# syncdoth/face_mask_inpaint

Measured on AMD Instinct MI355X. Metric: train images/sec at 256x256 bs=8 per GPU (PICNet-ref train step), higher is better.
Workload: dtype f32; 1 GPU; train_reference_fill.py PICNet-ref 256x256 fp32, bs=8 per GPU, synthetic CelebA-HQ-shaped batch + random binary_map (BASELINE configs[1]); global_batch=8, parallelism=dp1

## Files before the change

face_mask_inpaint_amd/csrc/conv.hip:

```cpp
#include "gemm_core.h"
#include "conv3x3.h"
#include "conv_p3.h"
#include "convt3x3.h"

static bool aligned16(const void* p) { return ((uintptr_t)p & 15) == 0; }
static int ep_vec(const ConvEp& ep, int Nout) {
  return Nout % 4 == 0 && ep.cstride % 4 == 0 && aligned16(ep.y) && aligned16(ep.bias) && aligned16(ep.res) && aligned16(ep.mask);
}

static int check_desc(const fmi_conv_desc* d) {
  if (!d) return FMI_ERR_BAD_ARG;
  if (d->N <= 0 || d->H <= 0 || d->W <= 0 || d->C <= 0 || d->K <= 0 || d->kh <= 0 || d->kw <= 0 || d->stride <= 0 ||
      d->pad < 0 || d->x_cstride < d->C || d->y_cstride < d->K)
    return FMI_ERR_BAD_ARG;
  const int pe = d->pad, dl = d->dil > 1 ? d->dil : 1;
  if (d->dil < 0 || (dl > 1 && d->pad_mode)) return FMI_ERR_BAD_ARG;
  if (d->OH != (d->H + 2 * pe - dl * (d->kh - 1) - 1) / d->stride + 1 || d->OW != (d->W + 2 * pe - dl * (d->kw - 1) - 1) / d->stride + 1)
    return FMI_ERR_BAD_ARG;
  if (d->OH <= 0 || d->OW <= 0) return FMI_ERR_BAD_ARG;
  if (d->pad_mode == 1 && (d->pad >= d->H || d->pad >= d->W)) return FMI_ERR_UNSUPPORTED;
  if (d->pad_mode != 0 && d->pad_mode != 1) return FMI_ERR_UNSUPPORTED;
  if ((int64_t)d->N * d->H * d->W > 0x7fffffffLL / 2 || (int64_t)d->kh * d->kw * d->C > 0x3fffffffLL) return FMI_ERR_UNSUPPORTED;
  return FMI_OK;
}

static ConvGeom fwd_geom(const fmi_conv_desc* d, const float* x, int n_eff) {
  ConvGeom g{};
  g.N = n_eff; g.IH = d->H; g.IW = d->W; g.C = d->C; g.cstride = d->x_cstride;
  g.GH = d->OH; g.GW = d->OW; g.S = d->stride;
  const int dl = d->dil > 1 ? d->dil : 1;
  g.nty = d->kh; g.ntx = d->kw; g.dy0 = -d->pad; g.dx0 = -d->pad; g.ystep = dl; g.xstep = dl;
  g.kh0 = 0; g.kw0 = 0; g.khstep = 1; g.kwstep = 1; g.kw = d->kw;
  g.pad_mode = d->pad_mode;
  g.vec = (d->C % 4 == 0) && (d->x_cstride % 4 == 0) && aligned16(x);
  g.dGW = make_fastdiv(g.GW); g.dG = make_fastdiv(g.GH * g.GW); g.dC = make_fastdiv(g.C); g.dntx = make_fastdiv(g.ntx);
  g.img_bs = (int64_t)d->H * d->W * d->x_cstride;
  return g;
}

static ConvGeom adj_geom(const fmi_conv_desc* d, const float* dy, int n_eff, int py, int px) {
  const int s = d->stride, dl = d->dil > 1 ? d->dil : 1;
  ConvGeom g{};
  g.N = n_eff; g.IH = d->OH; g.IW = d->OW; g.C = d->K; g.cstride = d->y_cstride;
  g.GH = (d->H - py + s - 1) / s; g.GW = (d->W - px + s - 1) / s; g.S = 1;
  g.kh0 = (py + d->pad) % s; g.kw0 = (px + d->pad) % s;
  g.nty = g.kh0 < d->kh ? (d->kh - g.kh0 + s - 1) / s : 0;
  g.ntx = g.kw0 < d->kw ? (d->kw - g.kw0 + s - 1) / s : 0;
  g.dy0 = (py + d->pad - g.kh0) / s; g.dx0 = (px + d->pad - g.kw0) / s;
  g.ystep = -dl; g.xstep = -dl; g.khstep = s; g.kwstep = s; g.kw = d->kw;
  g.pad_mode = 0;
  g.vec = (d->K % 4 == 0) && (d->y_cstride % 4 == 0) && aligned16(dy);
  g.dGW = make_fastdiv(g.GW); g.dG = make_fastdiv(g.GH * g.GW); g.dC = make_fastdiv(g.C);
  g.dntx = make_fastdiv(g.ntx > 0 ? g.ntx : 1);
  g.img_bs = (int64_t)d->OH * d->OW * d->y_cstride;
  if (g.nty == 0 || g.ntx == 0) { g.nty = 0; g.ntx = 1; }
  return g;
}

#ifndef FMI_HOST_EMU
__global__ void __launch_bounds__(256) conv_split_init_kernel(float* __restrict__ y, const float* __restrict__ bias,
                                                             const float* __restrict__ res, int K, int cstride, int64_t total) {
  for (int64_t i = (int64_t)blockIdx.x * 256 + threadIdx.x; i < total; i += (int64_t)gridDim.x * 256) {
    const int k = (int)(i % K);
    const int64_t o = (i / K) * cstride + k;
    float v = bias ? bias[k] : 0.f;
    if (res) v += res[o];
    y[o] = v;
  }
}
#endif

static int conv_ksplit(int64_t M, int N, int K) {
#ifdef FMI_HOST_EMU
  return 1;
#else
  const int64_t tiles = ceil_div64(M, 128) * ceil_div64(N, N <= 32 ? 32 : (N <= 64 ? 64 : 128));
  if (K < 512 || fmi_det()) return 1;
  if (tiles >= 320) {
    if (tiles >= 800 || K < 2304) return 1;
    return tiles <= 520 ? 2 : 3;
  }
  if (tiles >= 192 && K < 4608) return 1;
  int64_t ks = ceil_div64(384, tiles);
  const int64_t kmin = (M <= 128 && tiles <= 16) ? 64 : 256;
  if (ks > K / kmin) ks = K / kmin;
  return ks < 2 ? 1 : (int)(ks > (kmin == 64 ? 64 : 16) ? (kmin == 64 ? 64 : 16) : ks);
#endif
}

static int conv_phase(const fmi_conv_desc* d, const ConvGeom& g, const float* x, const void* x3, const float* w, const void* w3p,
                      int64_t w_bstride, int Nout, int flip, ConvEp ep, int batch_w, bool may_split, bool shared_init, hipStream_t st) {
  ConvK la{x, g};
  ConvWX lb{w, g, w_bstride, Nout, (Nout % 4 == 0) && aligned16(w) && (w_bstride % 4 == 0)};
  const int ks = may_split ? conv_ksplit(g.Mdim(), Nout, g.Kdim()) : 1;
#ifndef FMI_HOST_EMU
  if (shared_init || ks > 1) {
    if (!shared_init) {
      const int64_t total = (int64_t)g.N * ep.OHt * ep.OWt * Nout;
      hipLaunchKernelGGL(conv_split_init_kernel, dim3(fmi_bw_grid(total, 256)), dim3(256), 0, st, ep.y, ep.bias, ep.res, Nout, ep.cstride,
                         total);
    }
    ep.bias = nullptr;
    ep.res = nullptr;
    ep.act = 3;
    ep.vec = 0;
  }
  const uint16_t* w3 = (const uint16_t*)w3p;
  const int64_t w3_stride = (int64_t)d->kh * d->kw * d->C * d->K;
  const int64_t pixels = (int64_t)g.N * g.IH * g.IW;
  const bool tap3 = d->kh == 3 && d->kw == 3 && d->stride == 1 && d->pad == 1 && d->dil <= 1 && g.pad_mode == 0;
  const bool p3 = batch_w == 1 && g.cstride == g.C && g.Kdim() > 0 && p3_generic_ok(g, x3, w3, Nout);
  if (p3 && tap3 && conv3x3_p3_eligible(x3, w3, g.C, Nout, pixels)) {
    const C3P3Args ca{(const uint16_t*)x3, w3, g.N, g.IH, g.IW, g.C, Nout, flip, make_fastdiv(g.IW), make_fastdiv(g.IH * g.IW)};
    return launch_conv3x3_p3(ca, ep, g.Mdim(), ks, st);
  }
  if (p3)
    return launch_gemm_p3(ConvK3{(const uint16_t*)x3, g, make_fastdiv(g.ntaps())}, ConvWX3{w3, g, w3_stride, Nout}, ep, g.Mdim(), Nout,
                          g.Kdim(), ks, st);
  if (batch_w == 1 && tap3 && conv3x3_eligible(x, w, g.C, g.cstride, Nout, pixels)) {
    const C3Args ca{x, w, g.N, g.IH, g.IW, g.C, g.cstride, Nout, flip, make_fastdiv(g.IW), make_fastdiv(g.IH * g.IW), w3};
    return launch_conv3x3(ca, ep, g.Mdim(), ks, st);
  }
  if (w3 && la.dma_ok()) return launch_gemm(la, ConvWX3{w3, g, w3_stride, Nout}, ep, g.Mdim(), Nout, g.Kdim(), 1, ks, st);
#endif
  return launch_gemm(la, lb, ep, g.Mdim(), Nout, g.Kdim(), batch_w, ks, st);
}

static const void* weight_pieces(const fmi_conv_desc* d, int batch_w, int red_c) {
#ifndef FMI_HOST_EMU
  if (FMI_X6 && batch_w == 1 && red_c % 16 == 0 && aligned16(d->w3)) return d->w3;
#endif
  return nullptr;
}

static int check_y3(const fmi_conv_desc* d, int out_c, int out_cs) {
  if (!d->y3) return FMI_OK;
  return (out_c % 16 == 0 && out_cs == out_c && aligned16(d->y3)) ? FMI_OK : FMI_ERR_BAD_ARG;
}

extern "C" int fmi_conv2d_fwd_f32(const fmi_conv_desc* d, const float* x, const float* wf, const float* bias,
                                  const float* residual, float* y, int act, int batch_w, int64_t w_bstride,
                                  void* stream) {
  if (!d) return FMI_ERR_BAD_ARG;
  int rc = check_y3(d, d->K, d->y_cstride);
  if (rc) return rc;
  rc = check_desc(d);
  if (rc) return rc;
  if (!x || !wf || !y || batch_w < 1 || act < 0 || act > 2) return FMI_ERR_BAD_ARG;
  if (batch_w > 1 && batch_w != d->N) return FMI_ERR_BAD_ARG;
  auto finish = [&](int rc) {
#ifndef FMI_HOST_EMU
    if (rc == FMI_OK && d->y3) rc = fmi_split3_f32(y, d->y3, nullptr, (int64_t)d->N * d->OH * d->OW, d->K, 0, 0.f, stream);
#endif
    return rc;
  };
#ifndef FMI_HOST_EMU
  if (batch_w == 1 && fmi_conv2d_thin_supported(d) && aligned16(x))
    return finish(fmi_conv2d_thin_fwd_f32(d, x, wf, bias, residual, y, act, stream));
#endif
  const ConvGeom g = fwd_geom(d, x, batch_w > 1 ? 1 : d->N);
  const void* w3 = weight_pieces(d, batch_w, d->C);
  ConvEp ep{y, bias, residual, d->OH, d->OW, 1, 0, 0, d->OH, d->OW, d->y_cstride, act, g.dGW, g.dG, (int64_t)d->OH * d->OW * d->y_cstride};
  ep.vec = ep_vec(ep, d->K);
  return finish(conv_phase(d, g, x, d->x3, wf, w3, w_bstride, d->K, 0, ep, batch_w, act == 0 && batch_w == 1, false, (hipStream_t)stream));
}

static int dgrad_impl(const fmi_conv_desc* d, const float* dy, const float* wt, const float* bias, const float* residual,
                      const float* mask, float mslope, float* dx, int batch_w, int64_t w_bstride, void* stream) {
  if (!d) return FMI_ERR_BAD_ARG;
  int rc = check_y3(d, d->C, d->x_cstride);
  if (rc) return rc;
  rc = check_desc(d);
  if (rc) return rc;
  if (!dy || !wt || !dx || batch_w < 1) return FMI_ERR_BAD_ARG;
  if (d->pad_mode != 0) return FMI_ERR_UNSUPPORTED;
  if (batch_w > 1 && batch_w != d->N) return FMI_ERR_BAD_ARG;
  if (mask && bias) return FMI_ERR_UNSUPPORTED;
  auto finish = [&](int rc) {
#ifndef FMI_HOST_EMU
    if (rc == FMI_OK && d->y3) rc = fmi_split3_f32(dx, d->y3, nullptr, (int64_t)d->N * d->H * d->W, d->C, 0, 0.f, stream);
#endif
    return rc;
  };
#ifndef FMI_HOST_EMU
  if (batch_w == 1 && !bias && !residual && !mask && fmi_conv2d_thin_supported(d) && aligned16(dx))
    return finish(fmi_conv2d_thin_dgrad_f32(d, dy, wt, dx, stream));
  if (batch_w == 1 && !bias && !residual && !mask && d->C <= 4 && d->x_cstride == d->C) {
    const int rc_thin = fmi_conv2d_thin_input_dgrad_f32(d, dy, wt, dx, stream);
    if (rc_thin != FMI_ERR_UNSUPPORTED) return finish(rc_thin);
  }
#endif
  const int n_eff = batch_w > 1 ? 1 : d->N;
  const int s = d->stride;
  const void* w3 = weight_pieces(d, batch_w, d->K);
  if (d->dil > 1 && s != 1) return FMI_ERR_UNSUPPORTED;
  bool strided_split = false;
#ifndef FMI_HOST_EMU
  if (s > 1 && batch_w == 1) {
    for (int py = 0; py < s && !strided_split; ++py)
      for (int px = 0; px < s && !strided_split; ++px) {
        const ConvGeom g = adj_geom(d, dy, n_eff, py, px);
        if (g.GH > 0 && g.GW > 0 && conv_ksplit(g.Mdim(), d->C, g.Kdim()) > 1) strided_split = true;
      }
    if (strided_split) {
      const int64_t total = (int64_t)d->N * d->H * d->W * d->C;
      hipLaunchKernelGGL(conv_split_init_kernel, dim3(fmi_bw_grid(total, 256)), dim3(256), 0, (hipStream_t)stream, dx, bias, residual, d->C,
                         d->x_cstride, total);
    }
  }
  if (batch_w == 1 && !strided_split && !d->x3 && convt3x3_eligible(d, dy, (const uint16_t*)w3)) {
    CT3Args ca{};
    ca.x = dy; ca.w3 = (const uint16_t*)w3; ca.N = d->N; ca.H = d->OH; ca.W = d->OW; ca.Cred = d->K; ca.cs = d->y_cstride; ca.Nout = d->C;
    ca.dW = make_fastdiv(d->OW); ca.dHW = make_fastdiv(d->OH * d->OW);
    ConvEp ep{dx, bias, residual, d->OH, d->OW, 2, 0, 0, d->H, d->W, d->x_cstride, 0, ca.dW, ca.dHW, (int64_t)d->H * d->W * d->x_cstride};
    ep.mask = mask;
    ep.mslope = mslope;
    ep.vec = ep_vec(ep, d->C);
    ca.ep = ep;
    return finish(launch_convt3x3(ca, d->N * d->OH * d->OW, (hipStream_t)stream));
  }
#endif
  for (int py = 0; py < s; ++py) {
    for (int px = 0; px < s; ++px) {
      const ConvGeom g = adj_geom(d, dy, n_eff, py, px);
      if (g.GH <= 0 || g.GW <= 0) continue;
      ConvEp ep{dx, bias, residual, g.GH, g.GW, s, py, px, d->H, d->W, d->x_cstride, 0, g.dGW, g.dG,
                (int64_t)d->H * d->W * d->x_cstride};
      ep.mask = mask;
      ep.mslope = mslope;
      ep.vec = ep_vec(ep, d->C);
      rc = conv_phase(d, g, dy, d->x3, wt, w3, w_bstride, d->C, 1, ep, batch_w, batch_w == 1 && (s == 1 || strided_split), strided_split,
                      (hipStream_t)stream);
      if (rc) return rc;
    }
  }
  return finish(FMI_OK);
}
extern "C" int fmi_conv2d_dgrad_f32(const fmi_conv_desc* d, const float* dy, const float* wt, const float* bias,
                                    const float* residual, float* dx, int batch_w, int64_t w_bstride, void* stream) {
  return dgrad_impl(d, dy, wt, bias, residual, nullptr, 0.f, dx, batch_w, w_bstride, stream);
}
extern "C" int fmi_conv_transpose2d_pair_f32(const fmi_conv_desc* d, const float* x1, const float* x2, int K2, const void* w3b,
                                             const float* bias, float* y, void* stream) {
  int rc = check_desc(d);
  if (rc) return rc;
  if (!x1 || !x2 || !w3b || !d->w3 || !y || K2 <= 0) return FMI_ERR_BAD_ARG;
#ifndef FMI_HOST_EMU
  const uint16_t* w3 = (FMI_X6 && d->K % 16 == 0 && aligned16(d->w3)) ? (const uint16_t*)d->w3 : nullptr;
  if (!convt3x3_eligible(d, x1, w3) || (K2 & 15) || !aligned16(x2) || !aligned16(w3b) || d->pad_mode != 0 || d->x3) return FMI_ERR_UNSUPPORTED;
  CT3Args ca{};
  ca.x = x1; ca.w3 = w3; ca.x2 = x2; ca.w3b = (const uint16_t*)w3b; ca.Cred2 = K2; ca.cs2 = K2;
  ca.N = d->N; ca.H = d->OH; ca.W = d->OW; ca.Cred = d->K; ca.cs = d->y_cstride; ca.Nout = d->C;
  ca.dW = make_fastdiv(d->OW); ca.dHW = make_fastdiv(d->OH * d->OW);
  ConvEp ep{y, bias, nullptr, d->OH, d->OW, 2, 0, 0, d->H, d->W, d->x_cstride, 0, ca.dW, ca.dHW, (int64_t)d->H * d->W * d->x_cstride};
  ep.vec = ep_vec(ep, d->C);
  ca.ep = ep;
  return launch_convt3x3(ca, d->N * d->OH * d->OW, (hipStream_t)stream);
#else
  return FMI_ERR_UNSUPPORTED;
#endif
}
extern "C" int fmi_conv2d_dgrad_masked_f32(const fmi_conv_desc* d, const float* dy, const float* wt, const float* mask, float mask_slope,
                                           float* dx, void* stream) {
  if (!mask) return FMI_ERR_BAD_ARG;
  return dgrad_impl(d, dy, wt, nullptr, nullptr, mask, mask_slope, dx, 1, 0, stream);
}

extern "C" int fmi_conv2d_dgrad_masked_add_f32(const fmi_conv_desc* d, const float* dy, const float* wt, const float* mask, float mask_slope,
                                               const float* gadd, float* dx, void* stream) {
  if (!mask || !gadd) return FMI_ERR_BAD_ARG;
  return dgrad_impl(d, dy, wt, nullptr, gadd, mask, mask_slope, dx, 1, 0, stream);
}

extern "C" int fmi_conv2d_wgrad_f32(const fmi_conv_desc* d, const float* x, const float* dy, float* dwf, float* dbias,
                                    int batch_w, int64_t w_bstride, void* stream) {
  int rc = check_desc(d);
  if (rc) return rc;
  if (!x || !dy || !dwf || batch_w < 1) return FMI_ERR_BAD_ARG;
  if (batch_w > 1 && batch_w != d->N) return FMI_ERR_BAD_ARG;
#ifndef FMI_HOST_EMU
  if (batch_w == 1 && fmi_conv2d_thin_supported(d) && aligned16(x)) return fmi_conv2d_thin_wgrad_f32(d, x, dy, dwf, dbias, stream);
#endif
#ifndef FMI_HOST_EMU
  if (FMI_X6 && batch_w == 1 && !dbias && wgrad_p3_ok(d, d->x3, d->y3))
    return launch_wgrad_p3(d, (const uint16_t*)d->x3, (const uint16_t*)d->y3, dwf, (hipStream_t)stream);
#endif
  const int n_eff = batch_w > 1 ? 1 : d->N;
  ConvGeom g = fwd_geom(d, x, n_eff);
  const bool fuse_bias = dbias && batch_w == 1 && (g.Kdim() % 4 == 0);
  if (dbias && !fuse_bias) return FMI_ERR_UNSUPPORTED;
  const int ones_row = fuse_bias ? g.Kdim() : -1;
  const int Mg = g.Kdim() + (fuse_bias ? 1 : 0), Ng = d->K, Kg = g.Mdim();
  WgradAX la{x, g, ones_row};
  DenseX lb{dy, (int64_t)d->y_cstride, (int64_t)d->OH * d->OW * d->y_cstride, Ng, Kg,
            (d->K % 4 == 0) && (d->y_cstride % 4 == 0) && aligned16(dy)};
  WgradEp ep{dwf, g, d->K, w_bstride, dbias, ones_row};
  const int64_t tiles = ceil_div64(Mg, 128) * ceil_div64(Ng, Ng <= 32 ? 32 : (Ng <= 64 ? 64 : 128));
  int64_t ksplit = 2048 / (tiles * batch_w);
  const int64_t kmax = Kg / 512;
  if (ksplit > kmax) ksplit = kmax;
  if (ksplit < 1) ksplit = 1;
  if (fmi_det()) ksplit = 1;
  if (ksplit * batch_w > 65535) ksplit = 65535 / batch_w;
  return launch_gemm(la, lb, ep, Mg, Ng, Kg, batch_w, (int)ksplit, (hipStream_t)stream);
}

#ifndef FMI_HOST_EMU
__global__ void __launch_bounds__(256) bias_grad_vec_f64_kernel(const float* __restrict__ g, int64_t rows, int K4, float* __restrict__ dbias) {
  __shared__ double part[256][4];
  const int cg = threadIdx.x % K4, rl = threadIdx.x / K4, RL = 256 / K4;
  double s[4] = {0, 0, 0, 0};
  for (int64_t r = rl; r < rows; r += RL) {
    const float4 v = reinterpret_cast<const float4*>(g)[r * K4 + cg];
    s[0] += v.x, s[1] += v.y, s[2] += v.z, s[3] += v.w;
  }
#pragma unroll
  for (int e = 0; e < 4; ++e) part[threadIdx.x][e] = s[e];
  __syncthreads();
  if (threadIdx.x < K4) {
    double t[4] = {0, 0, 0, 0};
    for (int l = 0; l < RL; ++l)
#pragma unroll
      for (int e = 0; e < 4; ++e) t[e] += part[l * K4 + threadIdx.x][e];
#pragma unroll
    for (int e = 0; e < 4; ++e) atomicAdd(dbias + 4 * threadIdx.x + e, (float)t[e]);
  }
}
__global__ void __launch_bounds__(256) bias_grad_vec_kernel(const float* __restrict__ g, int64_t rows, int K4,
                                                            float* __restrict__ dbias, int64_t rows_per_block) {
  __shared__ float4 part[256];
  const int cg = threadIdx.x % K4, rl = threadIdx.x / K4, RL = 256 / K4;
  const int64_t r0 = (int64_t)blockIdx.x * rows_per_block;
  int64_t r1 = r0 + rows_per_block;
  if (r1 > rows) r1 = rows;
  float4 s = make_float4(0.f, 0.f, 0.f, 0.f);
  int64_t r = r0 + rl;
  for (; r + 3 * RL < r1; r += 4 * RL) {
    const float4 v0 = reinterpret_cast<const float4*>(g)[r * K4 + cg];
    const float4 v1 = reinterpret_cast<const float4*>(g)[(r + RL) * K4 + cg];
    const float4 v2 = reinterpret_cast<const float4*>(g)[(r + 2 * RL) * K4 + cg];
    const float4 v3 = reinterpret_cast<const float4*>(g)[(r + 3 * RL) * K4 + cg];
    s.x += (v0.x + v1.x) + (v2.x + v3.x);
    s.y += (v0.y + v1.y) + (v2.y + v3.y);
    s.z += (v0.z + v1.z) + (v2.z + v3.z);
    s.w += (v0.w + v1.w) + (v2.w + v3.w);
  }
  for (; r < r1; r += RL) {
    const float4 v = reinterpret_cast<const float4*>(g)[r * K4 + cg];
    s.x += v.x; s.y += v.y; s.z += v.z; s.w += v.w;
  }
  part[threadIdx.x] = s;
  __syncthreads();
  if (threadIdx.x < K4) {
    float4 t = part[threadIdx.x];
    for (int l = 1; l < RL; ++l) {
      const float4 v = part[l * K4 + threadIdx.x];
      t.x += v.x; t.y += v.y; t.z += v.z; t.w += v.w;
    }
    atomicAdd(dbias + 4 * threadIdx.x + 0, t.x);
    atomicAdd(dbias + 4 * threadIdx.x + 1, t.y);
    atomicAdd(dbias + 4 * threadIdx.x + 2, t.z);
    atomicAdd(dbias + 4 * threadIdx.x + 3, t.w);
  }
}
__global__ void __launch_bounds__(256) bias_grad_kernel(const float* __restrict__ g, int64_t rows, int K, int cstride,
                                                        float* __restrict__ dbias, int64_t rows_per_block) {
  __shared__ float part[4][64];
  const int tx = threadIdx.x & 63, ty = threadIdx.x >> 6;
  const int64_t r0 = (int64_t)blockIdx.x * rows_per_block;
  int64_t r1 = r0 + rows_per_block;
  if (r1 > rows) r1 = rows;
  for (int cg = 0; cg < K; cg += 64) {
    const int c = cg + tx;
    float s = 0.f;
    if (c < K)
      for (int64_t r = r0 + ty; r < r1; r += 4) s += g[r * cstride + c];
    part[ty][tx] = s;
    __syncthreads();
    if (ty == 0 && c < K) atomicAdd(dbias + c, part[0][tx] + part[1][tx] + part[2][tx] + part[3][tx]);
    __syncthreads();
  }
}

extern "C" int fmi_bias_grad_f32(const float* g, int64_t rows, int K, int cstride, float* dbias, void* stream) {
  if (!g || !dbias || rows <= 0 || K <= 0 || cstride < K) return FMI_ERR_BAD_ARG;
  int64_t blocks = ceil_div64(rows, 256);
  if (blocks > 256) blocks = 256;
  if (fmi_det()) blocks = 1;
  const int64_t rpb = ceil_div64(rows, blocks);
  blocks = ceil_div64(rows, rpb);
  const int K4 = K / 4;
  if (fmi_det() && K % 4 == 0 && cstride == K && K4 <= 256 && (K4 & (K4 - 1)) == 0 && (((uintptr_t)g) & 15) == 0)
    hipLaunchKernelGGL(bias_grad_vec_f64_kernel, dim3(1), dim3(256), 0, (hipStream_t)stream, g, rows, K4, dbias);
  else if (K % 4 == 0 && cstride == K && K4 <= 256 && (K4 & (K4 - 1)) == 0 && (((uintptr_t)g) & 15) == 0)
    hipLaunchKernelGGL(bias_grad_vec_kernel, dim3((unsigned)blocks), dim3(256), 0, (hipStream_t)stream, g, rows, K4, dbias, rpb);
  else
    hipLaunchKernelGGL(bias_grad_kernel, dim3((unsigned)blocks), dim3(256), 0, (hipStream_t)stream, g, rows, K, cstride, dbias, rpb);
  return fmi_launch_status();
}

__global__ void __launch_bounds__(256) reflect_fold_kernel(const float* __restrict__ gp, float* __restrict__ gx, int N,
                                                           int H, int W, int C, int pad, int64_t total) {
  const int HP = H + 2 * pad, WP = W + 2 * pad;
  for (int64_t i = (int64_t)blockIdx.x * 256 + threadIdx.x; i < total; i += (int64_t)gridDim.x * 256) {
    const int c = (int)(i % C);
    int64_t r = i / C;
    const int x = (int)(r % W);
    r /= W;
    const int y = (int)(r % H);
    const int n = (int)(r / H);
    int ys[3], xs[3], ny = 0, nx = 0;
    ys[ny++] = y + pad;
    if (y >= 1 && y <= pad) ys[ny++] = pad - y;
    if (y <= H - 2 && y >= H - 1 - pad) ys[ny++] = 2 * H - 2 - y + pad;
    xs[nx++] = x + pad;
    if (x >= 1 && x <= pad) xs[nx++] = pad - x;
    if (x <= W - 2 && x >= W - 1 - pad) xs[nx++] = 2 * W - 2 - x + pad;
    float s = 0.f;
    for (int a = 0; a < ny; ++a)
      for (int b = 0; b < nx; ++b) s += gp[(((int64_t)n * HP + ys[a]) * WP + xs[b]) * C + c];
    gx[i] = s;
  }
}

extern "C" int fmi_reflect_pad_fold_f32(const float* gpad, float* gx, int N, int H, int W, int C, int pad, void* stream) {
  if (!gpad || !gx || N <= 0 || H <= 0 || W <= 0 || C <= 0 || pad < 0 || pad >= H || pad >= W) return FMI_ERR_BAD_ARG;
  const int64_t total = (int64_t)N * H * W * C;
  hipLaunchKernelGGL(reflect_fold_kernel, dim3(fmi_bw_grid(total, 256)), dim3(256), 0, (hipStream_t)stream, gpad, gx, N,
                     H, W, C, pad, total);
  return fmi_launch_status();
}
#endif
```

face_mask_inpaint_amd/functional.py:

```python
from __future__ import annotations

import ctypes as C
import math
from typing import List, Optional, Sequence, Tuple

import torch

from . import _lib
from ._lib import ConvDesc, FmiError

EW_LRELU, EW_LRELU_BWD, EW_TANH_BWD, EW_ADD, EW_SCALE, EW_AXPY, EW_MUL, EW_RELU_BWD_OUT, EW_SOFTPLUS, EW_SOFTPLUS_BWD, EW_SUB, EW_RSQRT, EW_RSQRT_BWD, EW_SIGMOID, EW_SIGMOID_BWD = range(15)
ACT_NONE, ACT_TANH, ACT_RELU = 0, 1, 2

ATTN_CHUNK_BYTES = 96 * 1024 * 1024

PROFILE = None


class _prof:
    def __init__(self, tag, flops):
        self.tag, self.flops = tag, flops

    def __enter__(self):
        if PROFILE is not None:
# ... 52 lines not shown


def _p(t: Optional[torch.Tensor], off: int = 0):
    if t is None:
        return None
    return C.c_void_p(t.data_ptr() + 4 * off)


def _chk(*ts, dtype=torch.float32):
    for t in ts:
        if t is None:
            continue
        if not t.is_cuda:
            raise FmiError("face_mask_inpaint_amd ops need device tensors (there is no CPU fallback)")
        if t.dtype != dtype:
            raise FmiError(f"expected {dtype}, got {t.dtype}")
        if not t.is_contiguous():
            raise FmiError("expected a contiguous tensor")


class deterministic:

    def __init__(self, on: bool = True):
        self.on = bool(on)

    def __enter__(self):
        self.prev = _L().set_deterministic(1 if self.on else 0)
        return self

    def __exit__(self, *exc):
        _L().set_deterministic(self.prev)
        return False


def to_nhwc(x: torch.Tensor) -> torch.Tensor:
    return x.permute(0, 2, 3, 1).contiguous()


def to_nchw(x: torch.Tensor) -> torch.Tensor:
    return x.permute(0, 3, 1, 2)


def gemm_raw(a_ptr, b_ptr, c_ptr, M, N, K, sa, sb, sc, batch=1, bs=(0, 0, 0), alpha=1.0, beta=0.0, bias=None, tag="gemm"):
    with _prof(f"{tag}|{M}x{N}x{K} b{batch}", 2.0 * M * N * K * batch):
        _L().gemm_f32(a_ptr, b_ptr, c_ptr, M, N, K, sa[0], sa[1], sb[0], sb[1], sc[0], sc[1], batch, bs[0], bs[1], bs[2],
                      alpha, beta, _p(bias), _st())


def eltwise(op: int, a: torch.Tensor, b: Optional[torch.Tensor] = None, p0: float = 0.0, out: Optional[torch.Tensor] = None):
    _chk(a, b)
    y = torch.empty_like(a) if out is None else out
    if a.numel():
        _L().eltwise_f32(op, _p(a), _p(b), _p(y), a.numel(), float(p0), _st())
    return y


def conv_desc(n, h, w, c, k, kh, kw, stride, pad, pad_mode=0, x_cs=None, y_cs=None, dil=1, w3=None, x3=None) -> Tuple[ConvDesc, int, int]:
    oh = (h + 2 * pad - dil * (kh - 1) - 1) // stride + 1
    ow = (w + 2 * pad - dil * (kw - 1) - 1) // stride + 1
    d = ConvDesc(n, h, w, c, oh, ow, k, x_cs or c, y_cs or k, kh, kw, stride, pad, pad_mode, dil)
    if w3 is not None:
        d.w3 = w3.data_ptr()
        if x3 is not None:
            d.x3 = x3.data_ptr()
    return d, oh, ow


P3_ENABLED = True
P3_MIN_PIXELS = 16384
P3_MIN_WORK = 1152
P3_MIN_COUT = 64


def p3_wanted(pixels: int, cred: int, cout: int, taps: int) -> bool:
    return P3_ENABLED and cred % 16 == 0 and cred >= 64 and cout >= P3_MIN_COUT and pixels >= P3_MIN_PIXELS and taps * cout >= P3_MIN_WORK


def p3_of(t: torch.Tensor, lrelu_from: Optional[torch.Tensor] = None, slope: float = 0.0, colsum: Optional[list] = None) -> Optional[torch.Tensor]:
    c = t.shape[-1]
    if c % 16 or t.dtype != torch.float32 or not t.is_cuda or not t.is_contiguous() or t.data_ptr() % 16:
        if lrelu_from is not None:
            eltwise(EW_LRELU, lrelu_from, None, slope, out=t)
        return None
    p = getattr(t, "_fmi_p3", None)
    if p is not None and p[1] == t._version and lrelu_from is None:
        return p[0]
    x3 = torch.empty(t.numel() * 3, device=t.device, dtype=torch.bfloat16)
    if lrelu_from is not None:
        _L().split3_f32(_p(lrelu_from), C.c_void_p(x3.data_ptr()), _p(t), t.numel() // c, c, 1, float(slope), _st())
    elif colsum is not None and c <= 512 and 256 % (c // 8) == 0 and not _L().get_deterministic():
        gb = _zeros(c, t.device, torch.float32)
        _L().split3_colsum_f32(_p(t), C.c_void_p(x3.data_ptr()), _p(gb), t.numel() // c, c, _st())
        colsum.append(gb)
    else:
        _L().split3_f32(_p(t), C.c_void_p(x3.data_ptr()), None, t.numel() // c, c, 0, 0.0, _st())
    t._fmi_p3 = (x3, t._version)
    return x3


class PackedWeight:

    __slots__ = ("wf", "wt", "rows", "C", "kh", "kw", "w3")

    def __init__(self, wf, wt, rows, Cc, kh, kw, w3=(None, None)):
        self.wf, self.wt, self.rows, self.C, self.kh, self.kw = wf, wt, rows, Cc, kh, kw
        self.w3 = w3


W3_ENABLED = True
_LAST_W3: List[Tuple[Optional[torch.Tensor], Optional[torch.Tensor]]] = []


class _WeightPrepare(torch.autograd.Function):

    @staticmethod
    def forward(ctx, metas, *ws):
        lib = _L()
        n = len(ws)
        dev = ws[0].device
        sig = torch.ones(n, device=dev, dtype=torch.float32)
        entries = (_lib.WeightEntry * n)()
        wfs, wts, w3s = [], [], []
        for i, (w, meta) in enumerate(zip(ws, metas)):
            u, v = meta[0], meta[1]
            want_w3 = meta[2] if len(meta) > 2 else True
            iters = int(meta[3]) if len(meta) > 3 else 1
            _chk(w, u, v)
            rows, cc, kh, kw = w.shape
            if u is not None and rows > 4096:
                raise FmiError("spectral-norm weight with more than 4096 rows")
            wf = torch.empty((kh * kw, cc, rows), device=dev, dtype=torch.float32)
            wt = torch.empty((kh * kw, rows, cc), device=dev, dtype=torch.float32)
            pieces = W3_ENABLED and want_w3 and kh * kw <= 36 and w.is_cuda
            wf3 = torch.empty(3 * kh * kw * cc * rows, device=dev, dtype=torch.bfloat16) if pieces and cc % 16 == 0 else None
            wt3 = torch.empty(3 * kh * kw * cc * rows, device=dev, dtype=torch.bfloat16) if pieces and rows % 16 == 0 else None
            w3s.append((wf3, wt3))
            e = entries[i]
            e.wf3 = wf3.data_ptr() if wf3 is not None else None
            e.wt3 = wt3.data_ptr() if wt3 is not None else None
            e.w = w.data_ptr()
            e.u = u.data_ptr() if u is not None else None
            e.v = v.data_ptr() if v is not None else None
            e.wf, e.wt = wf.data_ptr(), wt.data_ptr()
            e.sigma = sig.data_ptr() + 4 * i
            e.rows, e.C, e.taps, e.iters = rows, cc, kh * kw, iters
            wfs.append(wf)
            wts.append(wt)
        lib.weight_prepare_f32(entries, n, _st())
        ctx.metas, ctx.ws, ctx.sig = metas, ws, sig
        _LAST_W3[:] = w3s
        ctx.mark_non_differentiable(sig, *wts)
        ctx.set_materialize_grads(False)
        return (sig,) + tuple(wfs) + tuple(wts)

    @staticmethod
    def backward(ctx, _gsig, *gs):
        lib = _L()
        n = len(ctx.ws)
        gwf = gs[:n]
        live = [i for i, g in enumerate(gwf) if g is not None and ctx.needs_input_grad[1 + i]]
        grads: List[Optional[torch.Tensor]] = [None] * n
        if live:
            entries = (_lib.WeightGradEntry * len(live))()
            keep = []
            for j, i in enumerate(live):
                w = ctx.ws[i]
                u, v = ctx.metas[i][0], ctx.metas[i][1]
                g = gwf[i].contiguous()
                dw = torch.empty_like(w)
                keep.append(g)
                e = entries[j]
                e.w = w.data_ptr()
                e.u = u.data_ptr() if u is not None else None
                e.v = v.data_ptr() if v is not None else None
                e.sigma = ctx.sig.data_ptr() + 4 * i
                e.dwf = g.data_ptr()
                e.dw = dw.data_ptr()
                e.rows, e.C, e.taps = w.shape[0], w.shape[1], w.shape[2] * w.shape[3]
                grads[i] = dw
            scratch = _zeros(len(live), ctx.sig.device, torch.float32)
            lib.weight_grad_f32(entries, len(live), _p(scratch), _st())
        return (None,) + tuple(grads)


def prepare_weights(items: Sequence[tuple]) -> List[PackedWeight]:
    metas = tuple(tuple(it[1:]) for it in items)
    ws = tuple(it[0] for it in items)
    n = len(ws)
    res = _WeightPrepare.apply(metas, *ws)
    w3s = list(_LAST_W3)
    _LAST_W3.clear()
    return [PackedWeight(res[1 + i], res[1 + n + i], w.shape[0], w.shape[1], w.shape[2], w.shape[3], w3s[i]) for i, w in enumerate(ws)]


def _act_bwd(g, y, act):
    if act == ACT_TANH:
        return eltwise(EW_TANH_BWD, g, y)
    if act == ACT_RELU:
        return eltwise(EW_RELU_BWD_OUT, g, y)
    return g


class _Conv2d(torch.autograd.Function):

    @staticmethod
    def forward(ctx, x, wf, bias, residual, wt, kh, kw, stride, pad, pad_mode, act, in_act=None, skip_act_bwd=False, dil=1, passthrough=False, w3=(None, None)):
        _chk(x, wf, bias, residual)
        lib = _L()
        x_in = x
        n, h, w, c = x.shape
        k = wf.shape[2]
        use3 = w3[0] is not None and pad_mode == 0 and p3_wanted(n * h * w, c, k, kh * kw)
        x3 = None
        if in_act is not None and in_act[0] == "apply":
            if use3:
                x = torch.empty_like(x_in)
                x3 = p3_of(x, lrelu_from=x_in, slope=in_act[1])
            else:
                x = eltwise(EW_LRELU, x, None, in_act[1])
        elif use3:
            x3 = p3_of(x)
        d, oh, ow = conv_desc(n, h, w, c, k, kh, kw, stride, pad, pad_mode, dil=dil, w3=w3[0], x3=x3)
        ctx.wt3 = w3[1]
        ctx.x3 = x3
        y = torch.empty((n, oh, ow, k), device=x.device, dtype=torch.float32)
        with _prof(f"conv_fwd|{n}x{h}x{w} {c}->{k} k{kh}s{stride}" + (f"d{dil}" if dil > 1 else ""), 2.0 * n * oh * ow * k * c * kh * kw):
            lib.conv2d_fwd_f32(C.byref(d), _p(x), _p(wf), _p(bias), _p(residual), _p(y), act, 1, 0, _st())
        ctx.save_for_backward(x, wf, y if (act and not skip_act_bwd) else None)
        ctx.wt, ctx.cfg, ctx.has = wt, (kh, kw, stride, pad, pad_mode, act), (bias is not None, residual is not None)
        ctx.dil = dil
        ctx.in_slope = None if in_act is None else float(in_act[1])
        ctx.skip_act_bwd = bool(skip_act_bwd)
        if passthrough:
            return y, x_in.view_as(x_in)
        return y

    @staticmethod
    def backward(ctx, gy, gpass=None):
        lib = _L()
        x, wf, y = ctx.saved_tensors
        if gy is None:
            return (gpass,) + (None,) * 15
        kh, kw, stride, pad, pad_mode, act = ctx.cfg
        gy = gy.contiguous()
        if act and not ctx.skip_act_bwd:
            gy = _act_bwd(gy, y, act)
        n, h, w, c = x.shape
        k = wf.shape[2]
        gx = gwf = gb = gres = None
        masked = False
        dil = ctx.dil
        gb_of_split = [] if (ctx.has[0] and ctx.needs_input_grad[2]) else None
        if ctx.needs_input_grad[0]:
            d0, _, _ = conv_desc(n, h, w, c, k, kh, kw, stride, pad, pad_mode, dil=dil)
            if pad_mode == 1 and lib.conv2d_thin_supported(C.byref(d0)):
                gx = torch.empty_like(x)
                with _prof(f"conv_dgrad|{n}x{h}x{w} {c}->{k} k{kh}s{stride}", 2.0 * gy.numel() * c * kh * kw):
                    lib.conv2d_thin_dgrad_f32(C.byref(d0), _p(gy), _p(ctx.wt), _p(gx), _st())
            elif pad_mode == 1:
                hp, wp = h + 2 * pad, w + 2 * pad
                d, _, _ = conv_desc(n, hp, wp, c, k, kh, kw, stride, 0, w3=ctx.wt3)
                gpad = torch.empty((n, hp, wp, c), device=x.device, dtype=torch.float32)
                with _prof(f"conv_dgrad|{n}x{h}x{w} {c}->{k} k{kh}s{stride}", 2.0 * gy.numel() * c * kh * kw):
                    lib.conv2d_dgrad_f32(C.byref(d), _p(gy), _p(ctx.wt), None, None, _p(gpad), 1, 0, _st())
                gx = torch.empty_like(x)
                lib.reflect_pad_fold_f32(_p(gpad), _p(gx), n, h, w, c, pad, _st())
            else:
                oh_, ow_ = gy.shape[1], gy.shape[2]
                gy3 = p3_of(gy, colsum=gb_of_split) if (ctx.wt3 is not None and p3_wanted(n * oh_ * ow_, k, c, kh * kw)) else None
                d, _, _ = conv_desc(n, h, w, c, k, kh, kw, stride, pad, dil=dil, w3=ctx.wt3, x3=gy3)
                gx = torch.empty_like(x)
                with _prof(f"conv_dgrad|{n}x{h}x{w} {c}->{k} k{kh}s{stride}", 2.0 * gy.numel() * c * kh * kw):
                    if ctx.in_slope is not None and gpass is not None:
                        lib.conv2d_dgrad_masked_add_f32(C.byref(d), _p(gy), _p(ctx.wt), _p(x), ctx.in_slope, _p(gpass.contiguous()), _p(gx), _st())
                        masked, gpass = True, None
                    elif ctx.in_slope is not None:
                        lib.conv2d_dgrad_masked_f32(C.byref(d), _p(gy), _p(ctx.wt), _p(x), ctx.in_slope, _p(gx), _st())
                        masked = True
                    elif gpass is not None:
                        lib.conv2d_dgrad_f32(C.byref(d), _p(gy), _p(ctx.wt), None, _p(gpass.contiguous()), _p(gx), 1, 0, _st())
                        gpass = None
                    else:
                        lib.conv2d_dgrad_f32(C.byref(d), _p(gy), _p(ctx.wt), None, None, _p(gx), 1, 0, _st())
            if ctx.in_slope is not None and not masked:
                gx = eltwise(EW_LRELU_BWD, gx, x, ctx.in_slope)
            if gpass is not None:
                gx = eltwise(EW_ADD, gx, gpass.contiguous())
        elif gpass is not None:
            gx = gpass
        if ctx.needs_input_grad[1]:
            d, _, _ = conv_desc(n, h, w, c, k, kh, kw, stride, pad, pad_mode, dil=dil)
            gwf = _zeros_like(wf)
            want_gb = ctx.has[0] and ctx.needs_input_grad[2]
            if ctx.x3 is not None and pad_mode == 0 and c % 32 == 0 and k % 16 == 0 and p3_wanted(gy.numel() // k, c, k, kh * kw):
                gy3 = p3_of(gy, colsum=gb_of_split)
                if gy3 is not None:
                    d.w3 = None
                    d.x3, d.y3 = ctx.x3.data_ptr(), gy3.data_ptr()
                    want_gb_fused = False
                else:
                    want_gb_fused = want_gb
            else:
                want_gb_fused = want_gb
            fuse = want_gb_fused and (kh * kw * c) % 4 == 0
            if fuse:
                gb = _zeros(k, x.device, torch.float32)
            with _prof(f"conv_wgrad|{n}x{h}x{w} {c}->{k} k{kh}s{stride}", 2.0 * gy.numel() * c * kh * kw):
                lib.conv2d_wgrad_f32(C.byref(d), _p(x), _p(gy), _p(gwf), _p(gb) if fuse else None, 1, 0, _st())
        if ctx.has[0] and ctx.needs_input_grad[2] and gb is None:
            if gb_of_split:
                gb = gb_of_split[0]
            else:
                gb = _zeros(k, x.device, torch.float32)
                lib.bias_grad_f32(_p(gy), gy.numel() // k, k, k, _p(gb), _st())
        if ctx.has[1] and ctx.needs_input_grad[3]:
            gres = gy
        return gx, gwf, gb, gres, None, None, None, None, None, None, None, None, None, None, None, None


class _ThinConvLReLU(torch.autograd.Function):

    @staticmethod
    def forward(ctx, x, wf, bias, wt, slope, pad_mode, act):
        _chk(x, wf, bias)
        n, h, w, c = x.shape
        k = wf.shape[2]
        d, oh, ow = conv_desc(n, h, w, c, k, 3, 3, 1, 1, pad_mode)
        y = torch.empty((n, oh, ow, k), device=x.device, dtype=torch.float32)
        with _prof(f"conv_fwd|{n}x{h}x{w} {c}->{k} k3s1", 2.0 * n * oh * ow * k * c * 9):
            _L().conv2d_thin_lrelu_fwd_f32(C.byref(d), _p(x), slope, _p(wf), _p(bias), _p(y), act, _st())
        ctx.save_for_backward(x, wf, y if act else None)
        ctx.wt, ctx.cfg, ctx.has_b = wt, (slope, pad_mode, act), bias is not None
        return y

    @staticmethod
    def backward(ctx, gy):
        lib = _L()
        x, wf, y = ctx.saved_tensors
        slope, pad_mode, act = ctx.cfg
        gy = gy.contiguous()
        if act:
            gy = _act_bwd(gy, y, act)
        n, h, w, c = x.shape
        k = wf.shape[2]
        d, _, _ = conv_desc(n, h, w, c, k, 3, 3, 1, 1, pad_mode)
        gx = gwf = gb = None
        if ctx.needs_input_grad[0]:
            gx = torch.empty_like(x)
            with _prof(f"conv_dgrad|{n}x{h}x{w} {c}->{k} k3s1", 2.0 * gy.numel() * c * 9):
                lib.conv2d_thin_lrelu_dgrad_f32(C.byref(d), _p(gy), _p(ctx.wt), _p(x), slope, _p(gx), _st())
        if ctx.needs_input_grad[1]:
            gwf = _zeros_like(wf)
            if ctx.has_b and ctx.needs_input_grad[2]:
                gb = _zeros(k, x.device, torch.float32)
            with _prof(f"conv_wgrad|{n}x{h}x{w} {c}->{k} k3s1", 2.0 * gy.numel() * c * 9):
                lib.conv2d_thin_lrelu_wgrad_f32(C.byref(d), _p(x), slope, _p(gy), _p(gwf), _p(gb), _st())
        elif ctx.has_b and ctx.needs_input_grad[2]:
            gb = _zeros(k, x.device, torch.float32)
            lib.bias_grad_f32(_p(gy), gy.numel() // k, k, k, _p(gb), _st())
        return gx, gwf, gb, None, None, None, None


def lrelu_conv2d(x, pw: PackedWeight, bias=None, slope=0.1, pad=1, pad_mode=0, act=ACT_NONE):
    if x.dtype == torch.float32 and pw.kh == 3 and pw.kw == 3 and pad == 1 and x.is_cuda:
        n, h, w, c = x.shape
        d, _, _ = conv_desc(n, h, w, c, pw.wf.shape[2], 3, 3, 1, 1, pad_mode)
        if _L().conv2d_thin_lrelu_supported(C.byref(d)) and x.data_ptr() % 16 == 0:
            return _ThinConvLReLU.apply(x, pw.wf, bias, pw.wt, float(slope), pad_mode, act)
    return conv2d(leaky_relu(x, slope), pw, bias, None, 1, pad, pad_mode, act)


def conv2d(x, pw: PackedWeight, bias=None, residual=None, stride=1, pad=0, pad_mode=0, act=ACT_NONE, in_act=None, skip_act_bwd=False, dilation=1,
           passthrough=False):
    if x.dtype == BF16:
        if bias is not None or residual is not None or pad_mode or act or in_act is not None or dilation != 1:
            raise FmiError("the bf16 convolution has no bias / residual / activation / reflect-padding / dilation form")
        return _Conv2dBF16.apply(x, pw.wf, pw.wt, pw.kh, pw.kw, stride, pad)
    return _Conv2d.apply(x, pw.wf, bias, residual, pw.wt, pw.kh, pw.kw, stride, pad, pad_mode, act, in_act, skip_act_bwd, int(dilation), bool(passthrough), pw.w3)


BF16 = torch.bfloat16


def _split_ws(out: torch.Tensor, kred: int):
    if out.numel() > (1 << 22) or kred < 1024:
        return None, 0
    ws = torch.zeros(out.numel(), device=out.device, dtype=torch.float32)
    return ws, ws.numel()


def _pack_bf16(src_tab: torch.Tensor) -> torch.Tensor:
    t, a, b = src_tab.shape
    out = torch.empty((b, t, a), device=src_tab.device, dtype=BF16)
    _L().pack_weight_bf16(_p(src_tab), _p(out), t, a, b, _st())
    return out


class _Conv2dBF16(torch.autograd.Function):

    @staticmethod
    def forward(ctx, x, wf, wt, kh, kw, stride, pad):
        _chk(x, dtype=BF16)
        _chk(wf, wt)
        lib = _L()
        n, h, w, c = x.shape
        k = wf.shape[2]
        d, oh, ow = conv_desc(n, h, w, c, k, kh, kw, stride, pad)
        y = torch.empty((n, oh, ow, k), device=x.device, dtype=BF16)
        wnk = _pack_bf16(wf)
        ws, wsn = _split_ws(y, c * kh * kw)
        with _prof(f"conv_fwd_bf16|{n}x{h}x{w} {c}->{k} k{kh}s{stride}", 2.0 * n * oh * ow * k * c * kh * kw):
            lib.conv2d_fwd_bf16(C.byref(d), _p(x), _p(wnk), None, _p(y), _p(ws), wsn, _st())
        ctx.save_for_backward(x, wf, wt)
        ctx.cfg = (kh, kw, stride, pad)
        return y

    @staticmethod
    def backward(ctx, gy):
        lib = _L()
        x, wf, wt = ctx.saved_tensors
        kh, kw, stride, pad = ctx.cfg
        gy = gy.contiguous()
        n, h, w, c = x.shape
        k = wf.shape[2]
        d, _, _ = conv_desc(n, h, w, c, k, kh, kw, stride, pad)
        gx = gwf = None
        if ctx.needs_input_grad[0]:
            gx = torch.empty_like(x)
            wck = _pack_bf16(wt)
            ws, wsn = _split_ws(gx, k * kh * kw)
            with _prof(f"conv_dgrad_bf16|{n}x{h}x{w} {c}->{k} k{kh}s{stride}", 2.0 * gy.numel() * c * kh * kw):
                lib.conv2d_dgrad_bf16(C.byref(d), _p(gy), _p(wck), None, _p(gx), _p(ws), wsn, _st())
        if ctx.needs_input_grad[1]:
            gwf = _zeros_like(wf)
            with _prof(f"conv_wgrad_bf16|{n}x{h}x{w} {c}->{k} k{kh}s{stride}", 2.0 * gy.numel() * c * kh * kw):
                lib.conv2d_wgrad_bf16(C.byref(d), _p(x), _p(gy), _p(gwf), _st())
        return gx, gwf, None, None, None, None, None


class _ConvTranspose2dBF16(torch.autograd.Function):

    @staticmethod
    def forward(ctx, x, wf, wt, kh, kw, stride, pad, out_pad):
        _chk(x, dtype=BF16)
        _chk(wf, wt)
        lib = _L()
        n, h, w, cs = x.shape
        cb = wf.shape[1]
        H = (h - 1) * stride - 2 * pad + kh + out_pad
        W = (w - 1) * stride - 2 * pad + kw + out_pad
        d, oh, ow = conv_desc(n, H, W, cb, cs, kh, kw, stride, pad)
        if (oh, ow) != (h, w):
            raise FmiError("unsupported ConvTranspose2d geometry")
        y = torch.empty((n, H, W, cb), device=x.device, dtype=BF16)
        wck = _pack_bf16(wt)
        ws, wsn = _split_ws(y, cs * kh * kw // (stride * stride))
        with _prof(f"convT_fwd_bf16|{n}x{h}x{w} {cs}->{cb}", 2.0 * x.numel() * cb * kh * kw):
            lib.conv2d_dgrad_bf16(C.byref(d), _p(x), _p(wck), None, _p(y), _p(ws), wsn, _st())
        ctx.save_for_backward(x, wf)
        ctx.cfg, ctx.HW = (kh, kw, stride, pad), (H, W)
        return y

    @staticmethod
    def backward(ctx, gy):
        lib = _L()
        x, wf = ctx.saved_tensors
        kh, kw, stride, pad = ctx.cfg
        H, W = ctx.HW
        gy = gy.contiguous()
        n, h, w, cs = x.shape
        cb = wf.shape[1]
        d, _, _ = conv_desc(n, H, W, cb, cs, kh, kw, stride, pad)
        gx = gwf = None
        if ctx.needs_input_grad[0]:
            gx = torch.empty_like(x)
            wnk = _pack_bf16(wf)
            ws, wsn = _split_ws(gx, cb * kh * kw)
            with _prof(f"convT_dgrad_bf16|{n}x{h}x{w} {cs}->{cb}", 2.0 * x.numel() * cb * kh * kw):
                lib.conv2d_fwd_bf16(C.byref(d), _p(gy), _p(wnk), None, _p(gx), _p(ws), wsn, _st())
        if ctx.needs_input_grad[1]:
            gwf = _zeros_like(wf)
            with _prof(f"convT_wgrad_bf16|{n}x{h}x{w} {cs}->{cb}", 2.0 * x.numel() * cb * kh * kw):
                lib.conv2d_wgrad_bf16(C.byref(d), _p(gy), _p(x), _p(gwf), _st())
        return gx, gwf, None, None, None, None, None, None


def _styled_out_bwd(g, y, noise, d, nw, bias, slope, gain, need_d, need_b, need_nw):
    n, c = y.shape[0], y.shape[-1]
    p = y.numel() // (n * c)
    t = torch.empty_like(y)
    gd = torch.empty((n, c), device=y.device, dtype=torch.float32) if (need_d and d is not None) else None
    gb = torch.empty(c, device=y.device, dtype=torch.float32) if (need_b and bias is not None) else None
    gnw = torch.empty(1, device=y.device, dtype=torch.float32) if (need_nw and noise is not None) else None
    ws = _parts_ws(y.device, max(2048, n) * 3 * c)
    sums = torch.empty(n * 3 * c, device=y.device, dtype=torch.float32)
    with _prof(f"bytes:noise_bias_act_fused_bwd|{tuple(y.shape)}", 3.0 * y.element_size() * y.numel()):
        _L().styled_out_bwd_bf16(_p(g), _p(y), _p(noise), _p(d), _p(nw), _p(bias), _p(t), _p(gd), _p(gb), _p(gnw), _p(ws), ws.numel(), _p(sums),
                                 n, p, c, slope, gain, _st())
    return t, gd, gb, gnw


class _StyledConvBF16(torch.autograd.Function):

    @staticmethod
    def forward(ctx, x, wf, wt, d, noise, nw, bias, kh, kw, pad, slope, gain):
        _chk(x, dtype=BF16)
        _chk(wf, wt, d, noise, nw, bias)
        lib = _L()
        n, h, w, c = x.shape
        k = wf.shape[2]
        dsc, oh, ow = conv_desc(n, h, w, c, k, kh, kw, 1, pad)
        y = torch.empty((n, oh, ow, k), device=x.device, dtype=BF16)
        wnk = _pack_bf16(wf)
        with _prof(f"conv_fwd_bf16|{n}x{h}x{w} {c}->{k} k{kh}s1 +out", 2.0 * n * oh * ow * k * c * kh * kw):
            lib.conv2d_fwd_act_bf16(C.byref(dsc), _p(x), _p(wnk), _p(d), _p(noise), _p(nw), _p(bias), slope, gain, _p(y), _st())
        ctx.save_for_backward(x, wf, wt, d, noise, nw, bias, y)
        ctx.cfg = (kh, kw, pad, slope, gain)
        return y

    @staticmethod
    def backward(ctx, g):
        lib = _L()
        x, wf, wt, d, noise, nw, bias, y = ctx.saved_tensors
        kh, kw, pad, slope, gain = ctx.cfg
        n, h, w, c = x.shape
        k = wf.shape[2]
        ni = ctx.needs_input_grad
        t, gd, gb, gnw = _styled_out_bwd(g.contiguous(), y, noise, d, nw, bias, slope, gain, ni[3], ni[6], ni[5])
        dsc, _, _ = conv_desc(n, h, w, c, k, kh, kw, 1, pad)
        gx = gwf = None
        if ni[0]:
            gx = torch.empty_like(x)
            wck = _pack_bf16(wt)
            ws, wsn = _split_ws(gx, k * kh * kw)
            with _prof(f"conv_dgrad_bf16|{n}x{h}x{w} {c}->{k} k{kh}s1", 2.0 * t.numel() * c * kh * kw):
                lib.conv2d_dgrad_bf16(C.byref(dsc), _p(t), _p(wck), None, _p(gx), _p(ws), wsn, _st())
        if ni[1]:
            gwf = _zeros_like(wf)
            with _prof(f"conv_wgrad_bf16|{n}x{h}x{w} {c}->{k} k{kh}s1", 2.0 * t.numel() * c * kh * kw):
                lib.conv2d_wgrad_bf16(C.byref(dsc), _p(x), _p(t), _p(gwf), _st())
        return gx, gwf, None, gd, None, gnw, gb, None, None, None, None, None


def styled_conv_fused_ok(x, pw: PackedWeight, pad) -> bool:
    if x.dtype != BF16 or not x.is_cuda:
        return False
    n, h, w, c = x.shape
    k = pw.wf.shape[2]
    oh, ow = h + 2 * pad - pw.kh + 1, w + 2 * pad - pw.kw + 1
    return c % 64 == 0 and k % 4 == 0 and k > 64 and pw.kh * pw.kw <= 32 and n * oh * ow >= 32768


def styled_conv(x, pw: PackedWeight, d, noise, nw, bias, slope, gain, pad):
    return _StyledConvBF16.apply(x, pw.wf, pw.wt, d, noise, nw, bias, pw.kh, pw.kw, int(pad), float(slope), float(gain))


class _BlurActBF16(torch.autograd.Function):

    @staticmethod
    def forward(ctx, u, kernel, d, noise, nw, bias, pad0, pad1, slope, gain):
        _chk(u, dtype=BF16)
        _chk(kernel, d, noise, nw, bias)
        n, h, w, c = u.shape
        oh, ow = h + pad0 + pad1 - 3, w + pad0 + pad1 - 3
        y = torch.empty((n, oh, ow, c), device=u.device, dtype=BF16)
        with _prof(f"bytes:upfirdn2d|{n}x{h}x{w}x{c} up1 down1 +out", float(u.element_size()) * (u.numel() + y.numel())):
            _L().blur_act_bf16(_p(u), _p(kernel), _p(y), n, h, w, c, pad0, pad1, pad0, pad1, _p(d), _p(noise), _p(nw), _p(bias), slope, gain, 1, _st())
        ctx.save_for_backward(kernel, d, noise, nw, bias, y)
        ctx.cfg = (pad0, pad1, slope, gain, (n, h, w, c))
        return y

    @staticmethod
    def backward(ctx, g):
        kernel, d, noise, nw, bias, y = ctx.saved_tensors
        pad0, pad1, slope, gain, (n, h, w, c) = ctx.cfg
        ni = ctx.needs_input_grad
        t, gd, gb, gnw = _styled_out_bwd(g.contiguous(), y, noise, d, nw, bias, slope, gain, ni[2], ni[5], ni[4])
        gu = None
        if ni[0]:
            oh, ow = y.shape[1], y.shape[2]
            gk = torch.flip(kernel, [0, 1]).contiguous()
            g0, g1 = 3 - pad0, h - oh + pad0
            gu = torch.empty((n, h, w, c), device=g.device, dtype=BF16)
            with _prof(f"bytes:upfirdn2d_bwd|{n}x{h}x{w}x{c} up1 down1", float(t.element_size()) * (t.numel() + gu.numel())):
                _L().blur_act_bf16(_p(t), _p(gk), _p(gu), n, oh, ow, c, g0, g1, g0, g1, None, None, None, None, 1.0, 1.0, 1, _st())
        return gu, None, gd, None, gnw, gb, None, None, None, None


def blur_act(u, kernel, pad, d, noise, nw, bias, slope, gain):
    return _BlurActBF16.apply(u, kernel.contiguous(), d, noise, nw, bias, int(pad[0]), int(pad[1]), float(slope), float(gain))


def _parts_ws(device, floats: int) -> torch.Tensor:
    return torch.empty(int(floats), device=device, dtype=torch.float32)


class _ToRGB(torch.autograd.Function):

    @staticmethod
    def forward(ctx, x, w, s, bias, skip):
        _chk(x, dtype=BF16)
        _chk(w, s, bias, skip)
        n, h, wd, c = x.shape
        out = torch.empty((n, h, wd, 3), device=x.device, dtype=torch.float32)
        _L().torgb_fwd_bf16(_p(x), _p(w), _p(s), _p(bias), _p(skip), _p(out), n, h * wd, c, _st())
        ctx.save_for_backward(x, w, s)
        ctx.has = (bias is not None, skip is not None)
# ... 1480 lines not shown
```

Before: 101.2 images/s.

## Add thin-input wgrad kernel and raise split-K for small weight-gradient GEMMs

```diff
diff --git a/face_mask_inpaint_amd/csrc/conv.hip b/face_mask_inpaint_amd/csrc/conv.hip
--- a/face_mask_inpaint_amd/csrc/conv.hip
+++ b/face_mask_inpaint_amd/csrc/conv.hip
@@ -272,6 +272,184 @@
   return dgrad_impl(d, dy, wt, nullptr, gadd, mask, mask_slope, dx, 1, 0, stream);
 }
 
+struct WgradThinIn {
+  const float* x;
+  const float* dy;
+  ConvGeom g;
+  int ycs, K4;
+  __host__ __device__ __forceinline__ int64_t row_off(int n, int gy, int i) const {
+    int iy = gy * g.S + g.dy0 + g.ystep * i;
+    if (g.pad_mode) iy = reflect_idx(iy, g.IH);
+    return (unsigned)iy < (unsigned)g.IH ? ((int64_t)n * g.IH + iy) * g.IW * g.cstride : -1;
+  }
+  __host__ __device__ __forceinline__ int64_t col_off(int gx, int j) const {
+    int ix = gx * g.S + g.dx0 + g.xstep * j;
+    if (g.pad_mode) ix = reflect_idx(ix, g.IW);
+    return (unsigned)ix < (unsigned)g.IW ? (int64_t)ix * g.cstride : -1;
+  }
+  __host__ __device__ __forceinline__ void decode(int p, int& n, int& gy, int& gx) const {
+    n = (int)fdiv((uint32_t)p, g.dG);
+    const int rem = p - n * g.GH * g.GW;
+    gy = (int)fdiv((uint32_t)rem, g.dGW);
+    gx = rem - gy * g.GW;
+  }
+};
+
+static bool wgrad_thin_in_ok(const fmi_conv_desc* d, const float* dy, int batch_w) {
+  const int K4 = d->K / 4;
+  return batch_w == 1 && d->C <= 4 && ((d->kh == 3 && d->kw == 3) || (d->kh == 1 && d->kw == 1)) && d->K % 4 == 0 && K4 <= 16 &&
+         (K4 & (K4 - 1)) == 0 && d->y_cstride % 4 == 0 && aligned16(dy);
+}
+
+#ifndef FMI_HOST_EMU
+template <int KW, int CC>
+__global__ void __launch_bounds__(512) wgrad_thin_in_kernel(WgradThinIn a, float* __restrict__ dw, float* __restrict__ dbias) {
+  constexpr int R = KW * CC, RB = 8;
+  __shared__ float red[8][RB][64];
+  const int P = a.g.Mdim(), K4 = a.K4, K = 4 * K4, i = blockIdx.y;
+  const int kg = threadIdx.x & (K4 - 1), pl = threadIdx.x / K4, PL = 512 / K4, step = gridDim.x * PL;
+  float acc[R + 1][4];
+#pragma unroll
+  for (int r = 0; r <= R; ++r) acc[r][0] = acc[r][1] = acc[r][2] = acc[r][3] = 0.f;
+  auto pixel = [&](int p) {
+    int n, gy, gx;
+    a.decode(p, n, gy, gx);
+    const float4 v = ldg4(a.dy + (int64_t)p * a.ycs + 4 * kg);
+    const int64_t ro = a.row_off(n, gy, i);
+    float e[R];
+#pragma unroll
+    for (int j = 0; j < KW; ++j) {
+      const int64_t co = a.col_off(gx, j);
+      const bool ok = ro >= 0 && co >= 0;
+      const float* q = a.x + (ok ? ro + co : 0);
+#pragma unroll
+      for (int c = 0; c < CC; ++c) e[j * CC + c] = ok ? q[c] : 0.f;
+    }
+#pragma unroll
+    for (int r = 0; r < R; ++r) {
+      acc[r][0] = fmaf(e[r], v.x, acc[r][0]);
+      acc[r][1] = fmaf(e[r], v.y, acc[r][1]);
+      acc[r][2] = fmaf(e[r], v.z, acc[r][2]);
+      acc[r][3] = fmaf(e[r], v.w, acc[r][3]);
+    }
+    acc[R][0] += v.x;
+    acc[R][1] += v.y;
+    acc[R][2] += v.z;
+    acc[R][3] += v.w;
+  };
+  int p = blockIdx.x * PL + pl;
+  for (; p + step < P; p += 2 * step) {
+    pixel(p);
+    pixel(p + step);
+  }
+  if (p < P) pixel(p);
+#pragma unroll
+  for (int r = 0; r <= R; ++r)
+#pragma unroll
+    for (int e = 0; e < 4; ++e)
+      for (int off = K4; off < 64; off <<= 1) acc[r][e] += __shfl_xor(acc[r][e], off, 64);
+  const int w = threadIdx.x >> 6, lane = threadIdx.x & 63;
+#pragma unroll
+  for (int r0 = 0; r0 <= R; r0 += RB) {
+    if (lane < K4) {
+#pragma unroll
+      for (int rr = 0; rr < RB; ++rr)
+        if (r0 + rr <= R) {
+#pragma unroll
+          for (int e = 0; e < 4; ++e) red[w][rr][4 * lane + e] = acc[r0 + rr][e];
+        }
+    }
+    __syncthreads();
+    for (int t = threadIdx.x; t < RB * K; t += 512) {
+      const int rr = t / K, ch = t - rr * K, r = r0 + rr;
+      if (r > R || (r == R && (!dbias || i != 0))) continue;
+      float s = 0.f;
+#pragma unroll
+      for (int ww = 0; ww < 8; ++ww) s += red[ww][rr][ch];
+      if (r == R) atomicAdd(dbias + ch, s);
+      else atomicAdd(dw + (int64_t)(i * R + r) * K + ch, s);
+    }
+    __syncthreads();
+  }
+}
+
+static int launch_wgrad_thin_in(const WgradThinIn& a, float* dw, float* dbias, hipStream_t st) {
+  const int PL = 512 / a.K4;
+  int64_t blocks = ceil_div64(a.g.Mdim(), (int64_t)PL * 16);
+  if (blocks > 256) blocks = 256;
+  if (fmi_det()) blocks = 1;
+  const dim3 grid((unsigned)blocks, (unsigned)a.g.nty);
+#define FMI_THIN_IN(KW, CC) hipLaunchKernelGGL((wgrad_thin_in_kernel<KW, CC>), grid, dim3(512), 0, st, a, dw, dbias)
+  switch (a.g.C + 4 * (a.g.ntx == 3)) {
+    case 1: FMI_THIN_IN(1, 1); break;
+    case 2: FMI_THIN_IN(1, 2); break;
+    case 3: FMI_THIN_IN(1, 3); break;
+    case 4: FMI_THIN_IN(1, 4); break;
+    case 5: FMI_THIN_IN(3, 1); break;
+    case 6: FMI_THIN_IN(3, 2); break;
+    case 7: FMI_THIN_IN(3, 3); break;
+    case 8: FMI_THIN_IN(3, 4); break;
+    default: return FMI_ERR_UNSUPPORTED;
+  }
+#undef FMI_THIN_IN
+  return fmi_launch_status();
+}
+#else
+static int launch_wgrad_thin_in(const WgradThinIn& a, float* dw, float* dbias, hipStream_t) {
+  const int P = a.g.Mdim(), K = 4 * a.K4, KH = a.g.nty, KW = a.g.ntx, CC = a.g.C;
+  for (int r = 0; r < KH * KW * CC; ++r) {
+    const int t = r / CC, c = r % CC, i = t / KW, j = t % KW;
+    for (int k = 0; k < K; ++k) {
+      double s = 0;
+      for (int p = 0; p < P; ++p) {
+        int n, gy, gx;
+        a.decode(p, n, gy, gx);
+        const int64_t ro = a.row_off(n, gy, i), co = a.col_off(gx, j);
+        if (ro >= 0 && co >= 0) s += (double)a.x[ro + co + c] * a.dy[(int64_t)p * a.ycs + k];
+      }
+      atomicAdd(dw + (int64_t)r * K + k, (float)s);
+    }
+  }
+  if (dbias)
+    for (int k = 0; k < K; ++k) {
+      double s = 0;
+      for (int p = 0; p < P; ++p) s += a.dy[(int64_t)p * a.ycs + k];
+      atomicAdd(dbias + k, (float)s);
+    }
+  return FMI_OK;
+}
+#endif
+
+static int64_t wgrad_small_ksplit(int Mg, int Ng, int64_t Kg, int64_t ksplit, int64_t tiles128) {
+#ifdef FMI_HOST_EMU
+  return ksplit;
+#else
+  auto cost = [&](int64_t ks, int64_t& wgs, int64_t& atomics) {
+    const int64_t kchunk = ceil_div64(ceil_div64(Kg, ks), 16) * 16, z = ceil_div64(Kg, kchunk);
+    int bm = 128, bn = 128;
+    switch (pick_gemm_tile(Mg, Ng, z)) {
+      case GemmTile::t128x32: bn = 32; break;
+      case GemmTile::t128x64: bn = 64; break;
+      case GemmTile::t64x64: bm = 64; bn = 64; break;
+      case GemmTile::t128x128: break;
+      case GemmTile::t64x128: bm = 64; break;
+      case GemmTile::t32x128: bm = 32; break;
+    }
+    wgs = ceil_div64(Mg, bm) * ceil_div64(Ng, bn) * z;
+    atomics = wgs * bm * bn;
+  };
+  int64_t wgs, atomics;
+  cost(ksplit, wgs, atomics);
+  if (wgs > 640 || atomics > 1600000) return ksplit;
+  while (2 * ksplit <= Kg / 32 && 2 * ksplit <= 2048 / tiles128) {
+    cost(2 * ksplit, wgs, atomics);
+    if (wgs > 640 || atomics > 1600000) break;
+    ksplit *= 2;
+  }
+  return ksplit;
+#endif
+}
+
 extern "C" int fmi_conv2d_wgrad_f32(const fmi_conv_desc* d, const float* x, const float* dy, float* dwf, float* dbias,
                                     int batch_w, int64_t w_bstride, void* stream) {
   int rc = check_desc(d);
@@ -287,7 +465,15 @@
 #endif
   const int n_eff = batch_w > 1 ? 1 : d->N;
   ConvGeom g = fwd_geom(d, x, n_eff);
+  if (wgrad_thin_in_ok(d, dy, batch_w)) return launch_wgrad_thin_in(WgradThinIn{x, dy, g, d->y_cstride, d->K / 4}, dwf, dbias, (hipStream_t)stream);
   const bool fuse_bias = dbias && batch_w == 1 && (g.Kdim() % 4 == 0);
+#ifndef FMI_HOST_EMU
+  if (dbias && !fuse_bias && batch_w == 1) {
+    const int rc_b = fmi_bias_grad_f32(dy, (int64_t)d->N * d->OH * d->OW, d->K, d->y_cstride, dbias, stream);
+    if (rc_b) return rc_b;
+    dbias = nullptr;
+  }
+#endif
   if (dbias && !fuse_bias) return FMI_ERR_UNSUPPORTED;
   const int ones_row = fuse_bias ? g.Kdim() : -1;
   const int Mg = g.Kdim() + (fuse_bias ? 1 : 0), Ng = d->K, Kg = g.Mdim();
@@ -301,6 +487,7 @@
   if (ksplit > kmax) ksplit = kmax;
   if (ksplit < 1) ksplit = 1;
   if (fmi_det()) ksplit = 1;
+  else if (batch_w == 1) ksplit = wgrad_small_ksplit(Mg, Ng, Kg, ksplit, tiles);
   if (ksplit * batch_w > 65535) ksplit = 65535 / batch_w;
   return launch_gemm(la, lb, ep, Mg, Ng, Kg, batch_w, (int)ksplit, (hipStream_t)stream);
 }
diff --git a/face_mask_inpaint_amd/functional.py b/face_mask_inpaint_amd/functional.py
--- a/face_mask_inpaint_amd/functional.py
+++ b/face_mask_inpaint_amd/functional.py
@@ -378,7 +378,7 @@
                     want_gb_fused = want_gb
             else:
                 want_gb_fused = want_gb
-            fuse = want_gb_fused and (kh * kw * c) % 4 == 0
+            fuse = want_gb_fused
             if fuse:
                 gb = _zeros(k, x.device, torch.float32)
             with _prof(f"conv_wgrad|{n}x{h}x{w} {c}->{k} k{kh}s{stride}", 2.0 * gy.numel() * c * kh * kw):
```

New measurement: 102.3 images/s (median of 6 runs). 1.1% higher.
